# idthanm/mpg

Hardware: NVIDIA B200
Metric: model state-steps/s (fwd+bwd, n=25) (higher is better)
Workload: dtype f32

## Files before the change

### mpg_b200/csrc/api.cu

```cuda
#include <cstdio>
#include <cstdlib>
#include <cstring>
#include <new>
#include <vector>

#include "mlp_kernels.cuh"
#include "model_kernels.cuh"
#include "tc_rollout.cuh"
#include "replay.cuh"

using namespace mpg;

namespace {

struct NetStore {
  float* flat = nullptr;
  float* W1p = nullptr;
  float* W2p = nullptr;
  float* W2Tp = nullptr;
  float* adam_m = nullptr;
  float* adam_v = nullptr;
  int in_dim = 0, out_dim = 0;
  bool set = false;
};
// ... 541 lines not shown
  CUDA_OK(ctx, cudaMemcpyAsync(ns.adam_m, m, n * sizeof(float), cudaMemcpyDeviceToDevice, st));
  CUDA_OK(ctx, cudaMemcpyAsync(ns.adam_v, v, n * sizeof(float), cudaMemcpyDeviceToDevice, st));
  return MPG_OK;
}

int mpg_polyak_update(mpg_ctx* ctx, int src_net, int dst_net, float tau, void* stream) {
  int rc = check_net(ctx, src_net);
  if (!rc) rc = check_net(ctx, dst_net);
  if (rc) return rc;
  NetStore &a = ctx->nets[src_net], &d = ctx->nets[dst_net];
  if (a.in_dim != d.in_dim || a.out_dim != d.out_dim) return fail(ctx, MPG_ERR_ARG, "polyak: nets differ in shape%s");
  cudaStream_t st = (cudaStream_t)stream;
  const int n = layout(ctx, a).total;
  polyak_kernel<<<(n + 255) / 256, 256, 0, st>>>(d.flat, a.flat, n, tau);
  ctx->launches++;
  CUDA_OK(ctx, cudaGetLastError());
  return repack(ctx, dst_net, st);
}

int mpg_get_weights(mpg_ctx* ctx, int net, float* const w[6], void* stream) {
  int rc = check_net(ctx, net);
  if (rc) return rc;
  cudaStream_t st = (cudaStream_t)stream;
  NetStore& ns = ctx->nets[net];
  const GradLayout L = layout(ctx, ns);
  const int hw = ctx->cfg.hidden;
  const int off[6] = {L.oW1, L.ob1, L.oW2, L.ob2, L.oW3, L.ob3};
  const int cnt[6] = {ns.in_dim * hw, hw, hw * hw, hw, hw * ns.out_dim, ns.out_dim};
  for (int i = 0; i < 6; ++i)
    CUDA_OK(ctx, cudaMemcpyAsync(w[i], ns.flat + off[i], cnt[i] * sizeof(float), cudaMemcpyDefault, st));
  return MPG_OK;
}

int mpg_policy_grad(mpg_ctx* ctx, const mpg_rollout_params* p, const float* obs, const float* noise, float* grad_out,
                    float* returns_out, void* stream) {
  if (!ctx || !p || !obs || !grad_out) return fail(ctx, MPG_ERR_ARG, "null argument to mpg_policy_grad%s");
  if (p->real_env || ctx->cfg.env == MPG_ENV_PATH_TRACKING_REAL) return fail(ctx, MPG_ERR_UNSUPPORTED, "the real environment is forward only%s");
  cudaStream_t st = (cudaStream_t)stream;
  RolloutArgs a;
  int rc = fill_rollout_args(ctx, p, a);
  if (rc) return rc;
  a.obs = obs; a.noise = noise; a.returns_out = returns_out;
  a.noise_mode = noise ? 1 : (p->use_philox ? 2 : 0);
  const int MB = p->rows * p->M;
  if (ctx->backend == MPG_BACKEND_TC) {
    const int ntiles = (MB + tc::ACT_ROWS - 1) / tc::ACT_ROWS;
    const int grid = ntiles < ctx->sms ? ntiles : ctx->sms;
    tc::TcArgs ta = tc_args(ctx, a, p->policy_net, p->q_net);
    ta.store_steps = p->full_bptt ? p->horizon + 1 : 1;
    const size_t need = (size_t)ntiles * ta.store_steps * tc::SLOT_BYTES;
    if (!tc_ensure_store(ctx->tc, need)) return fail(ctx, MPG_ERR_CUDA, "cudaMalloc of the dW operand store failed%s");
    ta.store = ctx->tc.store;
    ta.rec_hi_only = rec_hi_only(ctx, (long long)MB * ta.store_steps);
    if (!tc_ensure_h2store(ctx->tc, (size_t)ntiles * (p->horizon + 1) * 2 * tc::ACT_SPLIT))
      return fail(ctx, MPG_ERR_CUDA, "cudaMalloc of the h2 image store failed%s");
    ta.h2store = ctx->tc.h2store;
    ta.z_ckpt = ctx->tc.z_ckpt;
    ta.prof = ctx->prof;
    const int tail = ntiles % ctx->sms, full = ntiles - tail;
    const bool split = ctx->tail_overlap && ctx->aux && full > 0 && tail > 0 && !ctx->prof
                       && (long long)(ctx->sms - tail) * 4 >= (long long)(full / ctx->sms) * ctx->sms / 2;
    CUDA_OK(ctx, cudaMemsetAsync(ctx->partial, 0, (size_t)(split ? 2 : 1) * ctx->sms * ctx->partial_stride * sizeof(float), st));
    if (ctx->timing) cudaEventRecord(ctx->ev0, st);
    if (!split) {
      CUDA_OK(ctx, tc_launch_rollout<true>(ctx->cfg.env, ctx->act, ta, grid, st));
      if (ctx->timing) { cudaEventRecord(ctx->ev1, st); ctx->timed = 1; }
      launch_dw(ctx, ta, 0, ntiles, 0, ctx->sms, st);
      launch_reduce(ctx, p->policy_net, ctx->sms, grad_out, nullptr, st);
      ctx->launches += 3;
    } else {
      ta.tile0 = 0; ta.tile1 = full;
      CUDA_OK(ctx, tc_launch_rollout<true>(ctx->cfg.env, ctx->act, ta, ctx->sms, st));
      CUDA_OK(ctx, cudaEventRecord(ctx->ev_wave, st));
      tc::TcArgs tb = ta;
      tb.tile0 = full; tb.tile1 = ntiles;
      tb.r.partial = ctx->partial + (size_t)ctx->sms * ctx->partial_stride;
      CUDA_OK(ctx, tc_launch_rollout<true>(ctx->cfg.env, ctx->act, tb, tail, st));
      if (ctx->timing) { cudaEventRecord(ctx->ev1, st); ctx->timed = 1; }
      CUDA_OK(ctx, cudaStreamWaitEvent(ctx->aux, ctx->ev_wave, 0));
      launch_dw(ctx, ta, 0, full, 0, ctx->sms - tail, ctx->aux);
      CUDA_OK(ctx, cudaEventRecord(ctx->ev_aux, ctx->aux));
      launch_dw(ctx, ta, full, tail, ctx->sms, ctx->sms, st);
      CUDA_OK(ctx, cudaStreamWaitEvent(st, ctx->ev_aux, 0));
      launch_reduce(ctx, p->policy_net, 2 * ctx->sms, grad_out, nullptr, st);
      ctx->launches += 5;
    }
    CUDA_OK(ctx, cudaGetLastError());
    return MPG_OK;
  }
  const int ntiles = (MB + TILE_R - 1) / TILE_R;
  const int grid = ntiles < ctx->sms ? ntiles : ctx->sms;
  CUDA_OK(ctx, cudaMemsetAsync(ctx->partial, 0, (size_t)grid * ctx->partial_stride * sizeof(float), st));
  rc = launch_rollout<true>(ctx, a, grid, st, ctx->cfg.env);
  if (rc) return rc;
  launch_reduce(ctx, p->policy_net, grid, grad_out, nullptr, st);
  ctx->launches++;
  CUDA_OK(ctx, cudaGetLastError());
  return MPG_OK;
}

int mpg_rollout_forward(mpg_ctx* ctx, const mpg_rollout_params* p, const float* obs, const float* start_actions,
                        const float* noise, float* returns_out, float* traj_obs, float* traj_rew, float* traj_act,
                        void* stream) {
  if (!ctx || !p || !obs) return fail(ctx, MPG_ERR_ARG, "null argument to mpg_rollout_forward%s");
  cudaStream_t st = (cudaStream_t)stream;
  RolloutArgs a;
  int rc = fill_rollout_args(ctx, p, a);
// ... 465 lines not shown
```

### mpg_b200/csrc/tc_common.cuh

```cuda
#pragma once
#include <cuda_bf16.h>
#include <cuda_fp16.h>

#include "common.cuh"

namespace mpg {
namespace tc {

constexpr int H = 256;

__device__ __forceinline__ uint32_t smem_u32(const void* p) { return (uint32_t)__cvta_generic_to_shared(p); }

__device__ __forceinline__ void mbar_init(uint64_t* bar, uint32_t count) {
  asm volatile("mbarrier.init.shared::cta.b64 [%0], %1;" ::"r"(smem_u32(bar)), "r"(count));
}
__device__ __forceinline__ void mbar_arrive(uint64_t* bar) {
  asm volatile("mbarrier.arrive.shared::cta.b64 _, [%0];" ::"r"(smem_u32(bar)) : "memory");
}
__device__ __forceinline__ void mbar_expect_tx(uint64_t* bar, uint32_t bytes) {
  asm volatile("mbarrier.arrive.expect_tx.shared::cta.b64 _, [%0], %1;" ::"r"(smem_u32(bar)), "r"(bytes) : "memory");
}
__device__ __forceinline__ bool mbar_try(uint64_t* bar, uint32_t parity) {
  uint32_t ok;
  asm volatile(
      "{\n\t.reg .pred p;\n\t"
      "mbarrier.try_wait.parity.shared::cta.b64 p, [%1], %2, %3;\n\t"
      "selp.u32 %0, 1, 0, p;\n\t}" : "=r"(ok) : "r"(smem_u32(bar)), "r"(parity), "r"(0x989680) : "memory");
  return ok != 0;
}
static __device__ unsigned long long* g_wait_dbg = nullptr;
#ifndef MPG_WAIT_LIMIT_CYCLES
#define MPG_WAIT_LIMIT_CYCLES 4000000000ll
#endif
static inline bool wait_dbg_attach(unsigned long long* dev_ptr) {
  return cudaMemcpyToSymbol(g_wait_dbg, &dev_ptr, sizeof(dev_ptr)) == cudaSuccess;
}
static __device__ __noinline__ void mbar_timeout(int site, uint32_t parity) {
  if (g_wait_dbg) {
    const int w = (int)(threadIdx.x >> 5);
    const int k = w >= 20 ? 5 + (w & 1) : w / 4;
    volatile unsigned long long* r = g_wait_dbg + 4 + 4 * k;
    r[0] = (unsigned long long)site;
    r[1] = (unsigned long long)blockIdx.x;
    r[2] = (unsigned long long)threadIdx.x;
    r[3] = (unsigned long long)parity + 1ull;
    g_wait_dbg[0] = 1ull;
    __threadfence_system();
  }
}
__device__ __forceinline__ void mbar_wait(uint64_t* bar, uint32_t parity, int site = 0) {
  if (mbar_try(bar, parity)) return;
  const long long t0 = clock64();
  while (!mbar_try(bar, parity)) {
    if (clock64() - t0 > MPG_WAIT_LIMIT_CYCLES) {
      mbar_timeout(site, parity);
      const long long t1 = clock64();
      while (clock64() - t1 < 400000000ll) {}
      __trap();
    }
  }
}
#define MBAR_WAIT(bar, parity) mbar_wait((bar), (parity), __LINE__)
__device__ __forceinline__ float ex2_ftz(float x) {
  float y;
  asm("ex2.approx.ftz.f32 %0, %1;" : "=f"(y) : "f"(x));
  return y;
}
__device__ __forceinline__ float exp_fast(float x) { return ex2_ftz(x * 1.4426950408889634f); }
__device__ __forceinline__ void fence_barrier_init() { asm volatile("fence.mbarrier_init.release.cluster;" ::: "memory"); }
__device__ __forceinline__ void fence_proxy_async() { asm volatile("fence.proxy.async.shared::cta;" ::: "memory"); }

__device__ __forceinline__ void bulk_g2s(void* smem_dst, const void* gmem_src, uint32_t bytes, uint64_t* bar) {
  asm volatile("cp.async.bulk.shared::cluster.global.mbarrier::complete_tx::bytes [%0], [%1], %2, [%3];" ::"r"(
                   smem_u32(smem_dst)), "l"(gmem_src), "r"(bytes), "r"(smem_u32(bar)) : "memory");
}
__device__ __forceinline__ void bulk_s2g(void* gmem_dst, const void* smem_src, uint32_t bytes) {
  asm volatile("cp.async.bulk.global.shared::cta.bulk_group [%0], [%1], %2;" ::"l"(gmem_dst), "r"(smem_u32(smem_src)),
               "r"(bytes) : "memory");
}
__device__ __forceinline__ void bulk_commit() { asm volatile("cp.async.bulk.commit_group;" ::: "memory"); }
__device__ __forceinline__ void bulk_wait_read_all() { asm volatile("cp.async.bulk.wait_group.read 0;" ::: "memory"); }
__device__ __forceinline__ void bulk_wait_read_pending(int pending) {
  switch (pending) {
    case 3: asm volatile("cp.async.bulk.wait_group.read 3;" ::: "memory"); break;
    case 2: asm volatile("cp.async.bulk.wait_group.read 2;" ::: "memory"); break;
    case 1: asm volatile("cp.async.bulk.wait_group.read 1;" ::: "memory"); break;
    default: asm volatile("cp.async.bulk.wait_group.read 0;" ::: "memory"); break;
  }
}
__device__ __forceinline__ void bulk_wait_all() { asm volatile("cp.async.bulk.wait_group 0;" ::: "memory"); }

__device__ __forceinline__ void tmem_alloc(uint32_t* smem_result, uint32_t ncols) {
  asm volatile("tcgen05.alloc.cta_group::1.sync.aligned.shared::cta.b32 [%0], %1;" ::"r"(smem_u32(smem_result)), "r"(ncols)
               : "memory");
  asm volatile("tcgen05.relinquish_alloc_permit.cta_group::1.sync.aligned;" ::: "memory");
}
__device__ __forceinline__ void tmem_dealloc(uint32_t taddr, uint32_t ncols) {
  asm volatile("tcgen05.dealloc.cta_group::1.sync.aligned.b32 %0, %1;" ::"r"(taddr), "r"(ncols) : "memory");
}
__device__ __forceinline__ void tc_fence_before() { asm volatile("tcgen05.fence::before_thread_sync;" ::: "memory"); }
__device__ __forceinline__ void tc_fence_after() { asm volatile("tcgen05.fence::after_thread_sync;" ::: "memory"); }

__device__ __forceinline__ void umma_bf16(uint32_t d_tmem, uint64_t a_desc, uint64_t b_desc, uint32_t idesc,
                                          uint32_t accumulate) {
  asm volatile(
      "{\n\t.reg .pred p;\n\t"
      "setp.ne.b32 p, %4, 0;\n\t"
      "tcgen05.mma.cta_group::1.kind::f16 [%0], %1, %2, %3, p;\n\t}" ::"r"(d_tmem), "l"(a_desc), "l"(b_desc), "r"(idesc),
      "r"(accumulate) : "memory");
}
__device__ __forceinline__ void umma_commit(uint64_t* bar) {
  asm volatile("tcgen05.commit.cta_group::1.mbarrier::arrive::one.shared::cluster.b64 [%0];" ::"r"(smem_u32(bar)) : "memory");
}

__device__ __forceinline__ void tmem_ld32(uint32_t taddr, float (&v)[32]) {
  uint32_t r[32];
  asm volatile(
      "tcgen05.ld.sync.aligned.32x32b.x32.b32 "
      "{%0, %1, %2, %3, %4, %5, %6, %7, %8, %9, %10, %11, %12, %13, %14, %15, "
      "%16, %17, %18, %19, %20, %21, %22, %23, %24, %25, %26, %27, %28, %29, %30, %31}, [%32];"
      : "=r"(r[0]), "=r"(r[1]), "=r"(r[2]), "=r"(r[3]), "=r"(r[4]), "=r"(r[5]), "=r"(r[6]), "=r"(r[7]), "=r"(r[8]),
        "=r"(r[9]), "=r"(r[10]), "=r"(r[11]), "=r"(r[12]), "=r"(r[13]), "=r"(r[14]), "=r"(r[15]), "=r"(r[16]),
        "=r"(r[17]), "=r"(r[18]), "=r"(r[19]), "=r"(r[20]), "=r"(r[21]), "=r"(r[22]), "=r"(r[23]), "=r"(r[24]),
        "=r"(r[25]), "=r"(r[26]), "=r"(r[27]), "=r"(r[28]), "=r"(r[29]), "=r"(r[30]), "=r"(r[31])
      : "r"(taddr));
  asm volatile("tcgen05.wait::ld.sync.aligned;" ::: "memory");
#pragma unroll
  for (int i = 0; i < 32; ++i) v[i] = __uint_as_float(r[i]);
}
__device__ __forceinline__ void tmem_ld16(uint32_t taddr, float (&v)[16]) {
  uint32_t r[16];
  asm volatile(
      "tcgen05.ld.sync.aligned.32x32b.x16.b32 "
// ... 91 lines not shown
```

### mpg_b200/csrc/tc_kernels.cuh

```cuda
#pragma once
#include "env_models.cuh"
#include "rollout_kernels.cuh"
#include "tc_gemm.cuh"

#ifndef MPG_EPI_INLINE
#define MPG_EPI_INLINE __forceinline__
#endif

namespace mpg {
namespace tc {

struct TcNet {
  const uint8_t* big_fwd;
  const uint8_t* big_dx;
  const uint8_t* l1;
  const uint8_t* l1b;
  const uint8_t* in;
  const float* W3;
  const float* b2;
  const float* b3;
  int in_dim, out_dim;
};

constexpr int BIAS_K = 15;
constexpr size_t SLOT_H1 = 0, SLOT_D2 = 131072, SLOT_P = 262144;
constexpr size_t SLOT_BYTES = 270336;

struct TcArgs {
  RolloutArgs r;
  TcNet pol, q;
  float* act_ckpt;
  float* z_ckpt;
  uint8_t* h2store;
  uint8_t* store;
  int store_steps;
  int rec_hi_only;
  int tile0, tile1;
  int q_regress;
  const float* q_target;
  float q_inv_rows;
  long long* prof;
};

struct MiscF {
  float W3p[H * 2];
  float b2p[H];
  float W3q[H * 2];
  float b2q[H];
  float part[4 * 2 * ACT_ROWS];
  float d3s[2 * ACT_ROWS];
  float wsum[8];
  float b3[4];
};
static_assert(sizeof(MiscF) <= SmemMap::MISC_BYTES, "MISC region too small");

constexpr int SM_D3IMG = SmemMap::TOTAL;
constexpr int SM_TOTAL = SM_D3IMG + 8192;

__device__ __forceinline__ void epi_bar() { asm volatile("bar.sync 1, %0;" ::"n"(EPI_THREADS) : "memory"); }
__device__ __forceinline__ float elu_fast(float x) { return x > 0.f ? x : exp_fast(x) - 1.f; }
template <int ACT>
__device__ __forceinline__ float act_fast(float x) {
  if constexpr (ACT == MPG_ACT_RELU) return x > 0.f ? x : 0.f;
  else if constexpr (ACT == MPG_ACT_TANH) return tanhf(x);
  else return elu_fast(x);
}
template <int ACT>
__device__ __forceinline__ float times_act_grad_out(float g, float h) {
  if constexpr (ACT == MPG_ACT_RELU) return h > 0.f ? g : 0.f;
  else if constexpr (ACT == MPG_ACT_TANH) return g * fmaf(-h, h, 1.f);
  else return fmaf(g, fminf(h, 0.f), g);
}
template <int ACT>
__device__ __forceinline__ float act_grad_log2e(float z) {
  if constexpr (ACT == MPG_ACT_RELU) {
    return z > 0.f ? 1.f : 0.f;
  } else if constexpr (ACT == MPG_ACT_TANH) {
    const float e = ex2_ftz(-2.f * fabsf(z)), d = 1.f + e;
    return __fdividef(4.f * e, d * d);
  } else {
    return ex2_ftz(fminf(z, 0.f));
  }
}

__device__ __forceinline__ void act_load8(const uint8_t* act_hi, const uint8_t* act_lo, int r, int cc, float* x) {
  const uint32_t off = act_chunk_off(r, cc);
  const uint4 h = *reinterpret_cast<const uint4*>(act_hi + off);
  const uint4 l = *reinterpret_cast<const uint4*>(act_lo + off);
  const uint32_t hw[4] = {h.x, h.y, h.z, h.w}, lw[4] = {l.x, l.y, l.z, l.w};
#pragma unroll
  for (int i = 0; i < 4; ++i) {
    x[2 * i] = __uint_as_float(hw[i] << 16) + __uint_as_float(lw[i] << 16);
    x[2 * i + 1] = __uint_as_float(hw[i] & 0xFFFF0000u) + __uint_as_float(lw[i] & 0xFFFF0000u);
  }
}

__device__ __forceinline__ void store_image(bool elected, uint8_t* gdst, const uint8_t* ssrc, uint32_t bytes) {
  fence_proxy_async();
  epi_bar();
  if (elected) {
    bulk_s2g(gdst, ssrc, bytes);
    bulk_commit();
  }
}
__device__ __forceinline__ void store_image_follow(bool elected, Bars* b, const Sync& s, uint8_t* gdst, const uint8_t* ssrc,
                                                   bool hi_only = false) {
  if (elected) {
    const uint32_t par = (s.k_cnt - 1) & 1;
#pragma unroll
    for (int kb = 0; kb < 4; ++kb) {
      mbar_wait(&b->kb_done[kb], par, 20000 + __LINE__);
// ... 178 lines not shown
}

__device__ __forceinline__ void bar_arrive(int id, int count) { asm volatile("bar.arrive %0, %1;" ::"r"(id), "r"(count) : "memory"); }
__device__ __forceinline__ void bar_sync(int id, int count) { asm volatile("bar.sync %0, %1;" ::"r"(id), "r"(count) : "memory"); }
constexpr int BAR_PART = 2;
constexpr int BAR_D3 = 3;
constexpr int BAR_ROW = 4;
constexpr int ROW_THREADS = ACT_ROWS;
constexpr int XCHG_THREADS = EPI_THREADS + ROW_THREADS;

template <int ENV, bool BWD, int ACT, int ROLE>
__device__ __forceinline__ void run_rollout(const TcArgs& A, uint8_t* smem, Bars* b) {
  using E = Env<ENV>;
  constexpr int S = E::S, NA = E::A;
  const RolloutArgs& a = A.r;
  const int tid = threadIdx.x, warp = tid >> 5, lane = tid & 31;
  const int row = (warp & 3) * 32 + lane, hc = (warp >> 2) & 3;
  const bool rowthread = (ROLE == ROLE_ROW);
  const bool elected = (ROLE == ROLE_EPI) && tid == 0;
  const int MB = a.rows * a.M;
  const int ntiles = (MB + ACT_ROWS - 1) / ACT_ROWS;
  MiscF* mf = reinterpret_cast<MiscF*>(smem + SmemMap::MISC);
  uint8_t* act_img = smem + SmemMap::ACT;
  uint8_t* p_img = smem + SmemMap::PIMG;
  uint8_t* d3_img = smem + SM_D3IMG;
  const uint32_t tmem = b->tmem_base;
  const uint32_t tm_z1c = tmem + TM_Z1C, tm_work = tmem + TM_WORK, tm_gp = tmem + TM_GP, tm_d1 = tmem + TM_D1, tm_d3 = tmem + TM_D3;
  const uint32_t lane_off = (uint32_t)((warp & 3) * 32) << 16;
  const float cscale = -1.f / ((float)a.M * (float)a.global_rows);
  const bool store_dw = BWD && A.store != nullptr;
  Sync sy;
  bool d1_started = false, d3_started = false;
  bool d1_pending = false, any_dw = false;
  bool store_pending = false;
  uint32_t acc_issued = 0;
  auto acc_wait = [&]() {
    if (ROLE == ROLE_ROW && d1_pending) {
      mbar_wait(&b->acc_done, sy.acc_cnt & 1, 20000 + __LINE__);
      ++sy.acc_cnt;
    }
    d1_pending = false;
  };
  float db3acc[2] = {0.f, 0.f};
  int prof_t = -1;
  auto stamp = [&](int id) {
#ifdef MPG_DEBUG_PROBES
    if (A.prof && blockIdx.x == 0 && prof_t >= 0
        && ((ROLE == ROLE_EPI && tid == 0) || ROLE == ROLE_MMA || (ROLE == ROLE_ROW && tid == EPI_THREADS)))
      A.prof[(ROLE == ROLE_MMA ? 32 : (ROLE == ROLE_ROW ? 64 : 0)) + id] = clock64();
#else
    (void)id; (void)prof_t;
#endif
  };

  unsigned long long list_bits = 0ull, q_bits = 0ull;
#pragma unroll
  for (int k = 0; k < MPG_MAX_LIST; ++k)
    if (k < a.n_list && a.list[k] < 64) {
      list_bits |= 1ull << a.list[k];
      if (a.list_w[k] != 0.f) q_bits |= 1ull << a.list[k];
    }
  auto list_index = [&](int tt) {
    int kidx = -1;
    if (tt >= 64 || ((list_bits >> tt) & 1ull)) {
#pragma unroll
      for (int k = 0; k < MPG_MAX_LIST; ++k) if (k < a.n_list && a.list[k] == tt) kidx = k;
    }
    return kidx;
  };

  const int tile_end = A.tile1 > 0 && A.tile1 < ntiles ? A.tile1 : ntiles;
  for (int tile = A.tile0 + blockIdx.x; tile < tile_end; tile += gridDim.x) {
    const int grow = tile * ACT_ROWS + row;
    const bool valid = rowthread && grow < MB;
    const int m_idx = valid ? grow / a.rows : 0, i_idx = valid ? grow % a.rows : 0;
    const unsigned long long noise_row = (unsigned long long)m_idx * (unsigned long long)a.global_rows
                                         + (unsigned long long)(a.row_offset + i_idx);
    uint8_t* h2tile = (BWD && A.h2store) ? A.h2store + (size_t)tile * (size_t)(a.horizon + 1) * (2 * ACT_SPLIT) : nullptr;
    float s[S];
#pragma unroll
    for (int j = 0; j < S; ++j) s[j] = 0.f;
    if (valid) {
      float o[MPG_MAX_OBS];
#pragma unroll
      for (int i = 0; i < MPG_MAX_OBS; ++i) o[i] = i < a.obs_dim ? a.obs[(size_t)i_idx * a.obs_dim + i] : 0.f;
      E::reset(o, s);
    }
    float rsum = 0.f, gpow = 1.f;

    auto write_pimg = [&](const float* st, const float* act_or_null, bool f16, uint8_t* gimg = nullptr) {
      float o[MPG_MAX_OBS];
#pragma unroll
      for (int i = 0; i < MPG_MAX_OBS; ++i) o[i] = 0.f;
      E::get_obs(st, o, a.nfd);
#pragma unroll
      for (int kh = 0; kh < 2; ++kh) {
        float x[8];
#pragma unroll
        for (int e = 0; e < 8; ++e) {
          const int i = kh * 8 + e;
          float v = i < a.obs_dim ? o[i] * a.obs_scale[i] : 0.f;
          if (act_or_null) {
#pragma unroll
            for (int j = 0; j < NA; ++j)
              if (i == a.obs_dim + j) v = act_or_null[j];
          }
          x[e] = i == BIAS_K ? 1.f : v;
        }
        uint4 h, l;
        if (f16) {
          split2h(x[0], x[1], h.x, l.x); split2h(x[2], x[3], h.y, l.y); split2h(x[4], x[5], h.z, l.z); split2h(x[6], x[7], h.w, l.w);
        } else {
          split2(x[0], x[1], h.x, l.x); split2(x[2], x[3], h.y, l.y); split2(x[4], x[5], h.z, l.z); split2(x[6], x[7], h.w, l.w);
        }
        const uint32_t off = p_chunk_off(row, kh);
        *reinterpret_cast<uint4*>(p_img + off) = h;
        *reinterpret_cast<uint4*>(p_img + off + P_LO) = l;
        if (gimg) {
          *reinterpret_cast<uint4*>(gimg + off) = h;
          *reinterpret_cast<uint4*>(gimg + off + P_LO) = l;
        }
      }
    };
    auto policy_forward = [&](float* zpre, uint8_t* h2slot, uint8_t* slot) {
      if (ROLE == ROLE_MMA) stamp(16);
#ifdef MPG_DEBUG_PROBES
      fwd_pair_issue<ROLE>(b, smem, sy, A.pol.l1, A.pol.big_fwd, tm_z1c, tm_work,
                           (ROLE == ROLE_MMA && A.prof && blockIdx.x == 0 && prof_t >= 0) ? A.prof + 96 : nullptr);
#else
      fwd_pair_issue<ROLE>(b, smem, sy, A.pol.l1, A.pol.big_fwd, tm_z1c, tm_work);
#endif
      if (ROLE == ROLE_MMA) stamp(17);
      if (ROLE == ROLE_EPI) {
        stamp(17);
        if (store_pending) { store_wait(elected); store_pending = false; }
        epi_hidden1_blocks<ACT>(b, tm_z1c + lane_off, act_img, row, hc);
        stamp(18);
        if (slot) { store_image_follow(elected, b, sy, slot + SLOT_H1, act_img, A.rec_hi_only != 0); store_pending = true; }
        epi_wait_d(b, sy);
        stamp(19);
        float p0, p1;
        if (BWD) epi_hidden2_gstore<ACT>(tm_work + lane_off, mf->b2p, mf->W3p, h2slot, row, hc, p0, p1);
        else epi_hidden2<ACT>(tm_work + lane_off, mf->b2p, mf->W3p, hc, p0, p1);
        stamp(20);
        mf->part[(hc * 2 + 0) * ACT_ROWS + row] = p0;
        mf->part[(hc * 2 + 1) * ACT_ROWS + row] = p1;
        bar_arrive(BAR_PART, XCHG_THREADS);
      }
      if (rowthread) {
        bar_sync(BAR_PART, XCHG_THREADS);
#pragma unroll
        for (int j = 0; j < NA; ++j)
          zpre[j] = mf->b3[j] + ((mf->part[(0 * 2 + j) * ACT_ROWS + row] + mf->part[(1 * 2 + j) * ACT_ROWS + row])
                                 + (mf->part[(2 * 2 + j) * ACT_ROWS + row] + mf->part[(3 * 2 + j) * ACT_ROWS + row]));
      }
    };
    auto q_forward = [&](bool with_img, uint8_t* qslot) -> float {
      float qv = 0.f;
      fwd_pair_issue<ROLE>(b, smem, sy, A.q.l1, A.q.big_fwd, tm_z1c, tm_work);
      if (ROLE == ROLE_EPI) {
        if (store_pending) { store_wait(elected); store_pending = false; }
        epi_hidden1_blocks<ACT>(b, tm_z1c + lane_off, act_img, row, hc);
        if (qslot) store_image(elected, qslot + SLOT_H1, act_img, A.rec_hi_only ? ACT_SPLIT : 2 * ACT_SPLIT);
        epi_wait_d(b, sy);
        float p0, p1;
        if (with_img) {
          if (qslot) store_wait(elected);
          epi_hidden2_img<ACT>(tm_work + lane_off, mf->b2q, mf->W3q, act_img, row, hc, p0, p1);
        } else {
          epi_hidden2<ACT>(tm_work + lane_off, mf->b2q, mf->W3q, hc, p0, p1);
        }
        mf->part[(hc * 2 + 0) * ACT_ROWS + row] = p0;
        bar_arrive(BAR_PART, XCHG_THREADS);
      }
      if (rowthread) {
        bar_sync(BAR_PART, XCHG_THREADS);
        qv = mf->b3[2] + ((mf->part[0 * ACT_ROWS + row] + mf->part[2 * ACT_ROWS + row])
                          + (mf->part[4 * ACT_ROWS + row] + mf->part[6 * ACT_ROWS + row]));
      }
      return qv;
    };

    acc_wait();
    for (int t = 0; t <= a.horizon; ++t) {
      float act[NA];
#pragma unroll
      for (int j = 0; j < NA; ++j) act[j] = 0.f;
      const bool given = (t == 0 && a.use_start_actions);
      const bool rec_f = store_dw && !A.q_regress && (a.full_bptt || t == 0);
      uint8_t* slot = rec_f ? A.store + ((size_t)tile * A.store_steps + (a.full_bptt ? t : 0)) * SLOT_BYTES : nullptr;
      if (tile == A.tile0 + (int)blockIdx.x && t == 2) {
        prof_t = t;
        if (ROLE != ROLE_MMA) stamp(16);
      } else if (prof_t >= 0) {
        if (ROLE != ROLE_MMA) stamp(22);
        prof_t = -1;
      }
      if (rowthread) {
        if (BWD && valid) {
          float* c = a.ckpt + ((size_t)t * MB + grow) * S;
#pragma unroll
          for (int j = 0; j < S; ++j) c[j] = s[j];
        }
        if (!given) write_pimg(s, nullptr, true);
      }
      if (!given) {
        float zpre[NA];
        policy_forward(zpre, BWD ? h2tile + (size_t)t * (2 * ACT_SPLIT) : nullptr, slot);
        stamp(21);
        if (rowthread) {
          float hg[NA];
#pragma unroll
          for (int j = 0; j < NA; ++j) head_fwd_grad(zpre[j], a.policy_out_tanh, a.action_range, act[j], hg[j]);
          if (BWD && valid)
#pragma unroll
            for (int j = 0; j < NA; ++j) {
              A.z_ckpt[((size_t)t * MB + grow) * (2 * NA) + j] = act[j];
              A.z_ckpt[((size_t)t * MB + grow) * (2 * NA) + NA + j] = hg[j];
            }
        }
      } else if (valid) {
#pragma unroll
        for (int j = 0; j < NA; ++j) act[j] = a.start_actions[(size_t)i_idx * NA + j];
      }
      if (valid && a.traj_act)
#pragma unroll
        for (int j = 0; j < NA; ++j) a.traj_act[((size_t)t * MB + grow) * NA + j] = act[j];
      const int kidx = list_index(t);
      if (kidx >= 0) {
        float qv = 0.f;
        if (BWD && valid)
#pragma unroll
          for (int j = 0; j < NA; ++j) A.act_ckpt[((size_t)kidx * MB + grow) * NA + j] = act[j];
        if (a.has_q) {
          if (rowthread) write_pimg(s, act, true);
          qv = q_forward(false, nullptr);
        }
        if (valid && a.returns_out)
#pragma unroll
          for (int k = 0; k < MPG_MAX_LIST; ++k)
            if (k < a.n_list && a.list[k] == t) a.returns_out[(size_t)k * MB + grow] = rsum + gpow * qv;
      }
      if (t < a.horizon && valid) {
        float eps = 0.f;
        if (E::HAS_NOISE) {
          if (a.noise_mode == 1) eps = a.noise[(size_t)t * MB + grow];
          else if (a.noise_mode == 2) eps = philox_normal(a.seed, noise_row, (uint32_t)t);
        }
        const float rew = E::step(s, act, eps, a.noise_mode != 0);
        const float prew = (rew + a.rew_shift) * a.rew_scale;
        rsum += gpow * prew;
        gpow *= a.gamma;
        if (a.traj_rew) a.traj_rew[(size_t)t * MB + grow] = prew;
        if (a.traj_obs) {
          float o[MPG_MAX_OBS];
          E::get_obs(s, o, a.nfd);
#pragma unroll
          for (int i = 0; i < MPG_MAX_OBS; ++i)
            if (i < a.obs_dim) a.traj_obs[((size_t)t * MB + grow) * a.obs_dim + i] = o[i];
        }
      }
    }
    if (BWD) {
      float lam[S], snext[S], spre[S], zpre_n[2 * NA];
#pragma unroll
      for (int j = 0; j < S; ++j) { lam[j] = 0.f; snext[j] = s[j]; spre[j] = s[j]; }
#pragma unroll
      for (int j = 0; j < 2 * NA; ++j)
        zpre_n[j] = (valid && !A.q_regress) ? A.z_ckpt[((size_t)a.horizon * MB + grow) * (2 * NA) + j] : 0.f;
      float w_later = 0.f;
      for (int t = a.horizon; t >= 0; --t) {
        if (t < a.horizon && list_index(t + 1) >= 0) {
#pragma unroll
          for (int k = 0; k < MPG_MAX_LIST; ++k) if (k < a.n_list && a.list[k] == t + 1) w_later += a.list_w[k];
        }
        float gp = 1.f;
        for (int i = 0; i < t; ++i) gp *= a.gamma;
        const bool want_dw = a.full_bptt || t == 0;
        const bool rec = store_dw && want_dw;
        prof_t = (tile == A.tile0 + (int)blockIdx.x && t == a.horizon - 2) ? t : -1;
        stamp(0);
        uint8_t* slot = rec ? A.store + ((size_t)tile * A.store_steps + (a.full_bptt ? t : 0)) * SLOT_BYTES : nullptr;
        float g_a[NA], g_s[S], act[NA], hgrad[NA];
#pragma unroll
        for (int j = 0; j < NA; ++j) { g_a[j] = 0.f; act[j] = zpre_n[j]; hgrad[j] = zpre_n[NA + j]; }
#pragma unroll
        for (int j = 0; j < S; ++j) g_s[j] = 0.f;
        if (valid) {
#pragma unroll
          for (int j = 0; j < S; ++j) s[j] = spre[j];
          if (t > 0) {
            const float* c = a.ckpt + ((size_t)(t - 1) * MB + grow) * S;
#pragma unroll
            for (int j = 0; j < S; ++j) spre[j] = c[j];
            if (!A.q_regress)
#pragma unroll
              for (int j = 0; j < 2 * NA; ++j) zpre_n[j] = A.z_ckpt[((size_t)(t - 1) * MB + grow) * (2 * NA) + j];
          }
        }
        if (ROLE == ROLE_ROW) stamp(4);
        const int kidx = list_index(t);
        if (want_dw) any_dw = true;
        float w_k = 0.f;
        if (kidx >= 0) {
#pragma unroll
          for (int k = 0; k < MPG_MAX_LIST; ++k) if (k < a.n_list && a.list[k] == t) w_k += a.list_w[k];
        }
        auto q_part_at = [&](int tt) {
          bool q = false;
          if (tt < 64) {
            q = (q_bits >> tt) & 1ull;
          } else {
#pragma unroll
            for (int k = 0; k < MPG_MAX_LIST; ++k) if (k < a.n_list && a.list[k] == tt && a.list_w[k] != 0.f) q = true;
          }
          return q && a.has_q;
        };
        const bool early = t < a.horizon && !q_part_at(t);
        const bool early_next = t > 0 && !q_part_at(t - 1) && !A.q_regress;
        auto load_h2 = [&](int tt) {
          const uint8_t* src = h2tile + (size_t)tt * (2 * ACT_SPLIT);
#pragma unroll
          for (int h = 0; h < 2; ++h) {
            mbar_wait(&b->img_empty[h], sy.i_cnt & 1, 20000 + __LINE__);
            mbar_expect_tx(&b->img_full[h], ACT_SPLIT);
#pragma unroll
            for (int sp = 0; sp < 2; ++sp)
#pragma unroll
              for (int k = 0; k < 2; ++k) {
                const size_t off = (size_t)sp * ACT_SPLIT + (size_t)(2 * h + k) * ACT_BLOCK;
                bulk_g2s(act_img + off, src + off, ACT_BLOCK, &b->img_full[h]);
              }
          }
        };
        if (kidx >= 0 && a.has_q && (q_part_at(t) || A.q_regress)) {
          const bool reg = A.q_regress != 0;
          uint8_t* qslot = (reg && store_dw) ? A.store + (size_t)tile * SLOT_BYTES : nullptr;
          if (rowthread) {
            float ak[NA];
#pragma unroll
            for (int j = 0; j < NA; ++j) ak[j] = valid ? A.act_ckpt[((size_t)kidx * MB + grow) * NA + j] : 0.f;
            acc_wait();
            write_pimg(s, ak, true);
          }
          const float qv = q_forward(true, qslot);
          if (rowthread) {
            float ak[NA];
#pragma unroll
            for (int j = 0; j < NA; ++j) ak[j] = valid ? A.act_ckpt[((size_t)kidx * MB + grow) * NA + j] : 0.f;
            write_pimg(s, ak, false, qslot ? qslot + SLOT_P : nullptr);
            fence_proxy_async();
            mbar_arrive(&b->p_full);
          }
          if (rowthread) {
            const float up = !valid ? 0.f : (reg ? (qv - A.q_target[i_idx]) * A.q_inv_rows : cscale * w_k * gp);
            mf->d3s[row] = up;
            if (reg) {
              write_d3(d3_img, row, up, 0.f);
              db3acc[0] += up;
            }
            bar_arrive(BAR_D3, XCHG_THREADS);
          }
          if (reg) d3_issue<ROLE>(b, smem, sy, SM_D3IMG, d3_started, tm_d3);
          if (ROLE == ROLE_EPI) {
            if (reg) epi_wait_d(b, sy);
            bar_sync(BAR_D3, XCHG_THREADS);
          }
          gemm_issue<ROLE>(0, b, smem, sy, A.q.big_dx, tm_work);
          if (ROLE == ROLE_EPI) {
            epi_delta2_blocks<ACT>(b, mf->W3q, mf->d3s[row], 0.f, act_img, row, hc, reg ? &sy : nullptr);
            if (qslot) store_image(elected, qslot + SLOT_D2, act_img, A.rec_hi_only ? ACT_SPLIT : 2 * ACT_SPLIT);
            epi_wait_d(b, sy);
          }
          bwd_tail_issue<ROLE>(b, smem, sy, A.q.l1b, A.q.in, !reg, reg, d1_started, tm_z1c, tm_gp, tm_d1, true);
          if (ROLE == ROLE_EPI) {
            if (qslot) store_wait(elected);
            epi_delta1_blocks<ACT>(b, tm_work + lane_off, tm_z1c + lane_off, act_img, row, hc);
            if (!reg) epi_wait_d(b, sy);
          }
          if (reg) { d1_pending = true; ++acc_issued; }
          if (rowthread && !reg) {
            mbar_wait(&b->gp_full, sy.gp_cnt & 1, 20000 + __LINE__);
            ++sy.gp_cnt;
            tc_fence_after();
            float gin[16];
            read_gp(tm_gp + lane_off, gin);
            if (valid) {
              float go[MPG_MAX_OBS];
#pragma unroll
              for (int i = 0; i < MPG_MAX_OBS; ++i) go[i] = i < a.obs_dim ? gin[i] * a.obs_scale[i] : 0.f;
              E::obs_grad_to_state(s, go, a.nfd, g_s);
#pragma unroll
              for (int j = 0; j < NA; ++j)
#pragma unroll
                for (int i = 0; i < 16; ++i)
                  if (i == a.obs_dim + j) g_a[j] += gin[i];
            }
          }
        }
        if (A.q_regress) continue;
        if (rowthread) {
          tc_fence_before();
          stamp(5);
          if (t < a.horizon && valid) {
            env_step_bwd<ENV, true>(s, act, lam, cscale * w_later * gp * a.rew_scale, g_s, g_a, snext);
          }
          stamp(14);
          float d3[2] = {0.f, 0.f};
#pragma unroll
          for (int j = 0; j < NA; ++j) {
            d3[j] = valid ? g_a[j] * hgrad[j] : 0.f;
            mf->d3s[j * ACT_ROWS + row] = d3[j];
          }
          if (NA == 1) mf->d3s[ACT_ROWS + row] = 0.f;
          if (want_dw) {
            write_d3(d3_img, row, d3[0], d3[1]);
            db3acc[0] += d3[0]; db3acc[1] += d3[1];
          }
          bar_arrive(BAR_D3, XCHG_THREADS);
          stamp(2);
        }
        if (!early) {
          if (ROLE == ROLE_MMA) { umma_commit(&b->img_empty[0]); umma_commit(&b->img_empty[1]); }
          if (elected) {
            bulk_wait_read_all();
            mbar_arrive(&b->img_empty[0]);
            mbar_arrive(&b->img_empty[1]);
          }
          if (ROLE == ROLE_PRODUCER) load_h2(t);
        }
        store_pending = false;
        stamp(1);
        if (ROLE == ROLE_EPI) {
          mbar_wait(&b->img_full[0], sy.i_cnt & 1, 20000 + __LINE__);
          stamp(3);
        }
        ++sy.i_cnt;
        if (ROLE == ROLE_MMA) stamp(5);
        if (want_dw) d3_issue<ROLE>(b, smem, sy, SM_D3IMG, d3_started, tm_d3, true, A.rec_hi_only != 0);
        if (ROLE == ROLE_MMA) stamp(6);
        if (rowthread) {
          acc_wait();
          stamp(12);
          write_pimg(s, nullptr, false, rec ? slot + SLOT_P : nullptr);
          fence_proxy_async();
          mbar_arrive(&b->p_full);
          stamp(13);
        }
        if (ROLE == ROLE_EPI) {
          bar_sync(BAR_D3, XCHG_THREADS);
        }
        if (ROLE == ROLE_MMA) stamp(3);
        gemm_issue<ROLE>(0, b, smem, sy, A.pol.big_dx, tm_work);
        if (ROLE == ROLE_MMA) stamp(4);
        if (ROLE == ROLE_EPI) {
          stamp(6);
          epi_delta2_from_h2<ACT>(b, mf->W3p, mf->d3s[row], mf->d3s[ACT_ROWS + row], act_img, row, hc, (sy.i_cnt - 1) & 1,
                             want_dw ? &sy : nullptr);
          stamp(7);
          if (rec) store_image_follow(elected, b, sy, slot + SLOT_D2, act_img, A.rec_hi_only != 0);
          epi_wait_d(b, sy);
          stamp(8);
        }
        bwd_tail_issue<ROLE>(b, smem, sy, A.pol.l1b, A.pol.in, t > 0, want_dw, d1_started, tm_z1c, tm_gp, tm_d1, true, early_next);
        if (ROLE == ROLE_PRODUCER && early_next) load_h2(t - 1);
        if (ROLE == ROLE_EPI) {
          epi_delta1_blocks<ACT>(b, tm_work + lane_off, tm_z1c + lane_off, act_img, row, hc, rec, elected, early_next);
          stamp(9);
          if (t > 0) epi_wait_d(b, sy);
          stamp(10);
        }
        if (want_dw) { d1_pending = true; ++acc_issued; }
        if (t > 0 && rowthread) {
          mbar_wait(&b->gp_full, sy.gp_cnt & 1, 20000 + __LINE__);
          ++sy.gp_cnt;
          tc_fence_after();
          stamp(10);
          float gin[16];
          read_gp(tm_gp + lane_off, gin);
          if (valid) {
#pragma unroll
            for (int j = 0; j < S; ++j) { lam[j] = g_s[j]; snext[j] = s[j]; }
            float go[MPG_MAX_OBS];
#pragma unroll
            for (int i = 0; i < MPG_MAX_OBS; ++i) go[i] = i < a.obs_dim ? gin[i] * a.obs_scale[i] : 0.f;
            E::obs_grad_to_state(s, go, a.nfd, lam);
          }
        }
        stamp(11);
      }
    }
  }
  if (rowthread && BWD) {
    float s0 = db3acc[0], s1 = db3acc[1];
#pragma unroll
    for (int o = 16; o > 0; o >>= 1) { s0 += __shfl_xor_sync(0xffffffffu, s0, o); s1 += __shfl_xor_sync(0xffffffffu, s1, o); }
    if (lane == 0) { mf->wsum[(warp & 3) * 2] = s0; mf->wsum[(warp & 3) * 2 + 1] = s1; }
    bar_sync(BAR_ROW, ROW_THREADS);
    if (tid == EPI_THREADS) {
      const GradLayout L(A.pol.in_dim, A.pol.out_dim, H);
      float* partial = a.partial + (size_t)blockIdx.x * a.partial_stride;
      partial[L.ob3 + 0] = (mf->wsum[0] + mf->wsum[2]) + (mf->wsum[4] + mf->wsum[6]);
      if (NA > 1) partial[L.ob3 + 1] = (mf->wsum[1] + mf->wsum[3]) + (mf->wsum[5] + mf->wsum[7]);
    }
  }
  if (ROLE == ROLE_EPI && acc_issued > 0) mbar_wait(&b->acc_done, (acc_issued - 1) & 1, 20000 + __LINE__);
  if (ROLE == ROLE_EPI) {
    tc_fence_before();
    if (elected) bulk_wait_all();
    if (BWD) {
      const GradLayout L(A.pol.in_dim, A.pol.out_dim, H);
      float* partial = a.partial + (size_t)blockIdx.x * a.partial_stride;
      if (any_dw && hc == 0) {
        tc_fence_after();
        const int ncol3 = A.q_regress ? 1 : NA;
#pragma unroll
        for (int half = 0; half < 2; ++half) {
          const int f = half * 128 + row;
          float v[16], v2[16];
          tmem_ld16(tm_d1 + half * 32 + lane_off, v);
          tmem_ld16(tm_d1 + half * 32 + 16 + lane_off, v2);
#pragma unroll
          for (int i = 0; i < 16; ++i)
            if (i < A.pol.in_dim) partial[L.oW1 + (size_t)i * H + f] = v[i] + v2[i];
          partial[L.ob1 + f] = v[BIAS_K] + v2[BIAS_K];
          tmem_ld16(tm_d3 + half * 16 + lane_off, v);
#pragma unroll
          for (int j = 0; j < 2; ++j)
            if (j < ncol3) partial[L.oW3 + (size_t)f * A.pol.out_dim + j] = v[j] + v[2 + j];
        }
      }
    }
  }
}

constexpr int ROLLOUT_THREADS = EPI_THREADS + ROW_THREADS + 128;
constexpr int ROW_WARP0 = EPI_WARPS, PRODUCER_WARP = EPI_WARPS + 4, MMA_WARP = EPI_WARPS + 5;
constexpr int LAUNCH_REGS = 80, EPI_REGS = 80, ROW_REGS = 96, AUX_REGS = 64;
static_assert(EPI_THREADS * EPI_REGS + ROW_THREADS * ROW_REGS + 128 * AUX_REGS <= ROLLOUT_THREADS * LAUNCH_REGS,
              "setmaxnreg only redistributes the register pool of the CTA");

template <int ENV, bool BWD, int ACT>
__global__ void __launch_bounds__(ROLLOUT_THREADS, 1) tc_rollout_kernel(const __grid_constant__ TcArgs A) {
  extern __shared__ uint8_t smem_raw[];
// ... 36 lines not shown
```

Measured before the change: 635.5 million.

## Cache Q-net hidden images in forward and prefetch them in backward pass

During the forward rollout, the Q-network's second-layer hidden activations at list steps are now written to an extended global h2 store. The backward pass then reloads them by bulk copy and recomputes only the delta from h2, instead of rerunning the Q forward GEMMs at those steps. The image pipeline is restructured so every backward step, including Q steps, prefetches the next image early, and the weights for upcoming forward passes are warmed in L2. The change also adds debug-gated timing probes, and in exchange uses more global memory and adds proxy fences.

```diff
diff --git a/mpg_b200/csrc/api.cu b/mpg_b200/csrc/api.cu
--- a/mpg_b200/csrc/api.cu
+++ b/mpg_b200/csrc/api.cu
@@ -617,7 +617,7 @@
     if (!tc_ensure_store(ctx->tc, need)) return fail(ctx, MPG_ERR_CUDA, "cudaMalloc of the dW operand store failed%s");
     ta.store = ctx->tc.store;
     ta.rec_hi_only = rec_hi_only(ctx, (long long)MB * ta.store_steps);
-    if (!tc_ensure_h2store(ctx->tc, (size_t)ntiles * (p->horizon + 1) * 2 * tc::ACT_SPLIT))
+    if (!tc_ensure_h2store(ctx->tc, (size_t)ntiles * (p->horizon + 1 + p->n_list) * 2 * tc::ACT_SPLIT))
       return fail(ctx, MPG_ERR_CUDA, "cudaMalloc of the h2 image store failed%s");
     ta.h2store = ctx->tc.h2store;
     ta.z_ckpt = ctx->tc.z_ckpt;
diff --git a/mpg_b200/csrc/tc_common.cuh b/mpg_b200/csrc/tc_common.cuh
--- a/mpg_b200/csrc/tc_common.cuh
+++ b/mpg_b200/csrc/tc_common.cuh
@@ -69,6 +69,7 @@
 __device__ __forceinline__ float exp_fast(float x) { return ex2_ftz(x * 1.4426950408889634f); }
 __device__ __forceinline__ void fence_barrier_init() { asm volatile("fence.mbarrier_init.release.cluster;" ::: "memory"); }
 __device__ __forceinline__ void fence_proxy_async() { asm volatile("fence.proxy.async.shared::cta;" ::: "memory"); }
+__device__ __forceinline__ void fence_proxy_async_global() { asm volatile("fence.proxy.async.global;" ::: "memory"); }
 
 __device__ __forceinline__ void bulk_g2s(void* smem_dst, const void* gmem_src, uint32_t bytes, uint64_t* bar) {
   asm volatile("cp.async.bulk.shared::cluster.global.mbarrier::complete_tx::bytes [%0], [%1], %2, [%3];" ::"r"(
@@ -79,6 +80,9 @@
                "r"(bytes) : "memory");
 }
 __device__ __forceinline__ void bulk_commit() { asm volatile("cp.async.bulk.commit_group;" ::: "memory"); }
+__device__ __forceinline__ void prefetch_l2(const void* gsrc, uint32_t bytes) {
+  asm volatile("cp.async.bulk.prefetch.L2.global [%0], %1;" ::"l"(gsrc), "r"(bytes) : "memory");
+}
 __device__ __forceinline__ void bulk_wait_read_all() { asm volatile("cp.async.bulk.wait_group.read 0;" ::: "memory"); }
 __device__ __forceinline__ void bulk_wait_read_pending(int pending) {
   switch (pending) {
diff --git a/mpg_b200/csrc/tc_kernels.cuh b/mpg_b200/csrc/tc_kernels.cuh
--- a/mpg_b200/csrc/tc_kernels.cuh
+++ b/mpg_b200/csrc/tc_kernels.cuh
@@ -42,6 +42,12 @@
   long long* prof;
 };
 
+constexpr int ACCT_TILE0 = 0, ACCT_FWD0 = 1, ACCT_BWD0 = 2, ACCT_TILE1 = 3, ACCT_NS0 = 4, ACCT_NS1 = 5;
+constexpr int ACCT_FSTEP = 8, ACCT_FQ = 72, ACCT_BSTEP = 136, ACCT_BQ = 200, ACCT_BMID = 264;
+constexpr int PROF_ACCT = 128, PROF_ACCT_STRIDE = 336;
+constexpr int PROF_TILES = PROF_ACCT + 2 * 3 * PROF_ACCT_STRIDE, PROF_TILES_MAX = 16;
+constexpr int PROF_LONGLONGS = PROF_TILES + 2 * PROF_TILES_MAX * 4;
+
 struct MiscF {
   float W3p[H * 2];
   float b2p[H];
@@ -57,6 +63,11 @@
 constexpr int SM_D3IMG = SmemMap::TOTAL;
 constexpr int SM_TOTAL = SM_D3IMG + 8192;
 
+__device__ __forceinline__ unsigned long long globaltimer_ns() {
+  unsigned long long t;
+  asm volatile("mov.u64 %0, %%globaltimer;" : "=l"(t));
+  return t;
+}
 __device__ __forceinline__ void epi_bar() { asm volatile("bar.sync 1, %0;" ::"n"(EPI_THREADS) : "memory"); }
 __device__ __forceinline__ float elu_fast(float x) { return x > 0.f ? x : exp_fast(x) - 1.f; }
 template <int ACT>
@@ -341,6 +352,22 @@
     (void)id; (void)prof_t;
 #endif
   };
+#ifdef MPG_DEBUG_PROBES
+  const int acct_slot = !A.prof ? -1 : (blockIdx.x == 0 ? 0 : (blockIdx.x == gridDim.x / 2 ? 1 : -1));
+  const bool acct_thread = (ROLE == ROLE_EPI && tid == 0) || ROLE == ROLE_MMA || (ROLE == ROLE_ROW && tid == EPI_THREADS);
+  long long* acct = (acct_slot >= 0 && acct_thread)
+                        ? A.prof + PROF_ACCT + (acct_slot * 3 + (ROLE == ROLE_EPI ? 0 : (ROLE == ROLE_MMA ? 1 : 2))) * PROF_ACCT_STRIDE
+                        : nullptr;
+  bool acct_on = false;
+#endif
+  auto astamp = [&](int id) {
+#ifdef MPG_DEBUG_PROBES
+    if (acct && acct_on) acct[id] = clock64();
+#else
+    (void)id;
+#endif
+  };
+  auto astamp_step = [&](int base, int tt) { if (tt < 64) astamp(base + tt); };
 
   unsigned long long list_bits = 0ull, q_bits = 0ull;
 #pragma unroll
@@ -357,15 +384,45 @@
     }
     return kidx;
   };
+  auto q_part_at = [&](int tt) {
+    bool q = false;
+    if (tt < 64) {
+      q = (q_bits >> tt) & 1ull;
+    } else {
+#pragma unroll
+      for (int k = 0; k < MPG_MAX_LIST; ++k) if (k < a.n_list && a.list[k] == tt && a.list_w[k] != 0.f) q = true;
+    }
+    return q && a.has_q;
+  };
+  auto warm_fwd_l2 = [&](const TcNet& n) {
+    if (ROLE == ROLE_PRODUCER && BWD && !A.q_regress) {
+      for (int i = 0; i < BIG_STAGES; ++i) prefetch_l2(n.big_fwd + (size_t)i * STAGE_BYTES, STAGE_BYTES);
+      prefetch_l2(n.l1, STAGE_BYTES);
+    }
+  };
 
   const int tile_end = A.tile1 > 0 && A.tile1 < ntiles ? A.tile1 : ntiles;
   for (int tile = A.tile0 + blockIdx.x; tile < tile_end; tile += gridDim.x) {
+#ifdef MPG_DEBUG_PROBES
+    const int tile_i = (tile - A.tile0 - (int)blockIdx.x) / (int)gridDim.x;
+    acct_on = tile_i == (tile_end - A.tile0 - (int)blockIdx.x > (int)gridDim.x ? 1 : 0);
+    if (acct && acct_on) acct[ACCT_NS0] = (long long)globaltimer_ns();
+    if (acct_slot >= 0 && elected && tile_i < PROF_TILES_MAX) {
+      long long* tl = A.prof + PROF_TILES + (acct_slot * PROF_TILES_MAX + tile_i) * 4;
+      tl[0] = clock64();
+      tl[1] = (long long)globaltimer_ns();
+    }
+#endif
+    astamp(ACCT_TILE0);
     const int grow = tile * ACT_ROWS + row;
     const bool valid = rowthread && grow < MB;
     const int m_idx = valid ? grow / a.rows : 0, i_idx = valid ? grow % a.rows : 0;
     const unsigned long long noise_row = (unsigned long long)m_idx * (unsigned long long)a.global_rows
                                          + (unsigned long long)(a.row_offset + i_idx);
     uint8_t* h2tile = (BWD && A.h2store) ? A.h2store + (size_t)tile * (size_t)(a.horizon + 1) * (2 * ACT_SPLIT) : nullptr;
+    auto h2q_img = [&](int kk) {
+      return A.h2store + ((size_t)ntiles * (size_t)(a.horizon + 1) + (size_t)tile * a.n_list + kk) * (2 * ACT_SPLIT);
+    };
     float s[S];
 #pragma unroll
     for (int j = 0; j < S; ++j) s[j] = 0.f;
@@ -444,7 +501,7 @@
                                  + (mf->part[(2 * 2 + j) * ACT_ROWS + row] + mf->part[(3 * 2 + j) * ACT_ROWS + row]));
       }
     };
-    auto q_forward = [&](bool with_img, uint8_t* qslot) -> float {
+    auto q_forward = [&](bool with_img, uint8_t* qslot, uint8_t* h2slot = nullptr) -> float {
       float qv = 0.f;
       fwd_pair_issue<ROLE>(b, smem, sy, A.q.l1, A.q.big_fwd, tm_z1c, tm_work);
       if (ROLE == ROLE_EPI) {
@@ -456,6 +513,8 @@
         if (with_img) {
           if (qslot) store_wait(elected);
           epi_hidden2_img<ACT>(tm_work + lane_off, mf->b2q, mf->W3q, act_img, row, hc, p0, p1);
+        } else if (BWD && h2slot) {
+          epi_hidden2_gstore<ACT>(tm_work + lane_off, mf->b2q, mf->W3q, h2slot, row, hc, p0, p1);
         } else {
           epi_hidden2<ACT>(tm_work + lane_off, mf->b2q, mf->W3q, hc, p0, p1);
         }
@@ -471,7 +530,10 @@
     };
 
     acc_wait();
+    astamp(ACCT_FWD0);
     for (int t = 0; t <= a.horizon; ++t) {
+      astamp_step(ACCT_FSTEP, t);
+      if (t < a.horizon && q_part_at(t + 1)) warm_fwd_l2(A.q);
       float act[NA];
 #pragma unroll
       for (int j = 0; j < NA; ++j) act[j] = 0.f;
@@ -522,8 +584,9 @@
 #pragma unroll
           for (int j = 0; j < NA; ++j) A.act_ckpt[((size_t)kidx * MB + grow) * NA + j] = act[j];
         if (a.has_q) {
+          astamp_step(ACCT_FQ, t);
           if (rowthread) write_pimg(s, act, true);
-          qv = q_forward(false, nullptr);
+          qv = q_forward(false, nullptr, (BWD && h2tile && !A.q_regress && q_part_at(t)) ? h2q_img(kidx) : nullptr);
         }
         if (valid && a.returns_out)
 #pragma unroll
@@ -550,6 +613,7 @@
         }
       }
     }
+    astamp(ACCT_BWD0);
     if (BWD) {
       float lam[S], snext[S], spre[S], zpre_n[2 * NA];
 #pragma unroll
@@ -558,6 +622,35 @@
       for (int j = 0; j < 2 * NA; ++j)
         zpre_n[j] = (valid && !A.q_regress) ? A.z_ckpt[((size_t)a.horizon * MB + grow) * (2 * NA) + j] : 0.f;
       float w_later = 0.f;
+      auto bwd_img = [&](int tt) { return q_part_at(tt) ? h2q_img(list_index(tt)) : h2tile + (size_t)tt * (2 * ACT_SPLIT); };
+      auto load_img = [&](const uint8_t* src) {
+#pragma unroll
+        for (int h = 0; h < 2; ++h) {
+          mbar_wait(&b->img_empty[h], sy.i_cnt & 1, 20000 + __LINE__);
+          mbar_expect_tx(&b->img_full[h], ACT_SPLIT);
+#pragma unroll
+          for (int sp = 0; sp < 2; ++sp)
+#pragma unroll
+            for (int k = 0; k < 2; ++k) {
+              const size_t off = (size_t)sp * ACT_SPLIT + (size_t)(2 * h + k) * ACT_BLOCK;
+              bulk_g2s(act_img + off, src + off, ACT_BLOCK, &b->img_full[h]);
+            }
+        }
+      };
+      if (!A.q_regress) {
+        if (ROLE == ROLE_MMA) { umma_commit(&b->img_empty[0]); umma_commit(&b->img_empty[1]); }
+        if (ROLE == ROLE_EPI) {
+          fence_proxy_async_global();
+          epi_bar();
+        }
+        if (elected) {
+          bulk_wait_read_all();
+          mbar_arrive(&b->img_empty[0]);
+          mbar_arrive(&b->img_empty[1]);
+        }
+        store_pending = false;
+        if (ROLE == ROLE_PRODUCER) load_img(bwd_img(a.horizon));
+      }
       for (int t = a.horizon; t >= 0; --t) {
         if (t < a.horizon && list_index(t + 1) >= 0) {
 #pragma unroll
@@ -569,6 +662,11 @@
         const bool rec = store_dw && want_dw;
         prof_t = (tile == A.tile0 + (int)blockIdx.x && t == a.horizon - 2) ? t : -1;
         stamp(0);
+        astamp_step(ACCT_BSTEP, t);
+        if (t == 1 && tile + (int)gridDim.x < tile_end) {
+          warm_fwd_l2(A.pol);
+          if (q_part_at(0)) warm_fwd_l2(A.q);
+        }
         uint8_t* slot = rec ? A.store + ((size_t)tile * A.store_steps + (a.full_bptt ? t : 0)) * SLOT_BYTES : nullptr;
         float g_a[NA], g_s[S], act[NA], hgrad[NA];
 #pragma unroll
@@ -595,44 +693,23 @@
 #pragma unroll
           for (int k = 0; k < MPG_MAX_LIST; ++k) if (k < a.n_list && a.list[k] == t) w_k += a.list_w[k];
         }
-        auto q_part_at = [&](int tt) {
-          bool q = false;
-          if (tt < 64) {
-            q = (q_bits >> tt) & 1ull;
-          } else {
-#pragma unroll
-            for (int k = 0; k < MPG_MAX_LIST; ++k) if (k < a.n_list && a.list[k] == tt && a.list_w[k] != 0.f) q = true;
-          }
-          return q && a.has_q;
-        };
-        const bool early = t < a.horizon && !q_part_at(t);
-        const bool early_next = t > 0 && !q_part_at(t - 1) && !A.q_regress;
-        auto load_h2 = [&](int tt) {
-          const uint8_t* src = h2tile + (size_t)tt * (2 * ACT_SPLIT);
-#pragma unroll
-          for (int h = 0; h < 2; ++h) {
-            mbar_wait(&b->img_empty[h], sy.i_cnt & 1, 20000 + __LINE__);
-            mbar_expect_tx(&b->img_full[h], ACT_SPLIT);
-#pragma unroll
-            for (int sp = 0; sp < 2; ++sp)
-#pragma unroll
-              for (int k = 0; k < 2; ++k) {
-                const size_t off = (size_t)sp * ACT_SPLIT + (size_t)(2 * h + k) * ACT_BLOCK;
-                bulk_g2s(act_img + off, src + off, ACT_BLOCK, &b->img_full[h]);
-              }
-          }
-        };
+        const bool early_next = t > 0 && !A.q_regress;
         if (kidx >= 0 && a.has_q && (q_part_at(t) || A.q_regress)) {
           const bool reg = A.q_regress != 0;
           uint8_t* qslot = (reg && store_dw) ? A.store + (size_t)tile * SLOT_BYTES : nullptr;
-          if (rowthread) {
-            float ak[NA];
-#pragma unroll
-            for (int j = 0; j < NA; ++j) ak[j] = valid ? A.act_ckpt[((size_t)kidx * MB + grow) * NA + j] : 0.f;
+          float qv = 0.f;
+          if (reg) {
+            if (rowthread) {
+              float ak[NA];
+#pragma unroll
+              for (int j = 0; j < NA; ++j) ak[j] = valid ? A.act_ckpt[((size_t)kidx * MB + grow) * NA + j] : 0.f;
+              acc_wait();
+              write_pimg(s, ak, true);
+            }
+            qv = q_forward(true, qslot);
+          } else if (rowthread) {
             acc_wait();
-            write_pimg(s, ak, true);
-          }
-          const float qv = q_forward(true, qslot);
+          }
           if (rowthread) {
             float ak[NA];
 #pragma unroll
@@ -653,18 +730,22 @@
           if (reg) d3_issue<ROLE>(b, smem, sy, SM_D3IMG, d3_started, tm_d3);
           if (ROLE == ROLE_EPI) {
             if (reg) epi_wait_d(b, sy);
+            else mbar_wait(&b->img_full[0], sy.i_cnt & 1, 20000 + __LINE__);
             bar_sync(BAR_D3, XCHG_THREADS);
           }
+          if (!reg) ++sy.i_cnt;
           gemm_issue<ROLE>(0, b, smem, sy, A.q.big_dx, tm_work);
           if (ROLE == ROLE_EPI) {
-            epi_delta2_blocks<ACT>(b, mf->W3q, mf->d3s[row], 0.f, act_img, row, hc, reg ? &sy : nullptr);
+            if (reg) epi_delta2_blocks<ACT>(b, mf->W3q, mf->d3s[row], 0.f, act_img, row, hc, &sy);
+            else epi_delta2_from_h2<ACT>(b, mf->W3q, mf->d3s[row], 0.f, act_img, row, hc, (sy.i_cnt - 1) & 1);
             if (qslot) store_image(elected, qslot + SLOT_D2, act_img, A.rec_hi_only ? ACT_SPLIT : 2 * ACT_SPLIT);
             epi_wait_d(b, sy);
           }
-          bwd_tail_issue<ROLE>(b, smem, sy, A.q.l1b, A.q.in, !reg, reg, d1_started, tm_z1c, tm_gp, tm_d1, true);
+          bwd_tail_issue<ROLE>(b, smem, sy, A.q.l1b, A.q.in, !reg, reg, d1_started, tm_z1c, tm_gp, tm_d1, true, !reg);
+          if (ROLE == ROLE_PRODUCER && !reg) load_img(h2tile + (size_t)t * (2 * ACT_SPLIT));
           if (ROLE == ROLE_EPI) {
             if (qslot) store_wait(elected);
-            epi_delta1_blocks<ACT>(b, tm_work + lane_off, tm_z1c + lane_off, act_img, row, hc);
+            epi_delta1_blocks<ACT>(b, tm_work + lane_off, tm_z1c + lane_off, act_img, row, hc, false, elected, !reg);
             if (!reg) epi_wait_d(b, sy);
           }
           if (reg) { d1_pending = true; ++acc_issued; }
@@ -686,6 +767,7 @@
                   if (i == a.obs_dim + j) g_a[j] += gin[i];
             }
           }
+          astamp_step(ACCT_BQ, t);
         }
         if (A.q_regress) continue;
         if (rowthread) {
@@ -708,21 +790,13 @@
           }
           bar_arrive(BAR_D3, XCHG_THREADS);
           stamp(2);
-        }
-        if (!early) {
-          if (ROLE == ROLE_MMA) { umma_commit(&b->img_empty[0]); umma_commit(&b->img_empty[1]); }
-          if (elected) {
-            bulk_wait_read_all();
-            mbar_arrive(&b->img_empty[0]);
-            mbar_arrive(&b->img_empty[1]);
-          }
-          if (ROLE == ROLE_PRODUCER) load_h2(t);
-        }
-        store_pending = false;
+          astamp_step(ACCT_BMID, t);
+        }
         stamp(1);
         if (ROLE == ROLE_EPI) {
           mbar_wait(&b->img_full[0], sy.i_cnt & 1, 20000 + __LINE__);
           stamp(3);
+          astamp_step(ACCT_BMID, t);
         }
         ++sy.i_cnt;
         if (ROLE == ROLE_MMA) stamp(5);
@@ -739,7 +813,7 @@
         if (ROLE == ROLE_EPI) {
           bar_sync(BAR_D3, XCHG_THREADS);
         }
-        if (ROLE == ROLE_MMA) stamp(3);
+        if (ROLE == ROLE_MMA) { stamp(3); astamp_step(ACCT_BMID, t); }
         gemm_issue<ROLE>(0, b, smem, sy, A.pol.big_dx, tm_work);
         if (ROLE == ROLE_MMA) stamp(4);
         if (ROLE == ROLE_EPI) {
@@ -752,7 +826,7 @@
           stamp(8);
         }
         bwd_tail_issue<ROLE>(b, smem, sy, A.pol.l1b, A.pol.in, t > 0, want_dw, d1_started, tm_z1c, tm_gp, tm_d1, true, early_next);
-        if (ROLE == ROLE_PRODUCER && early_next) load_h2(t - 1);
+        if (ROLE == ROLE_PRODUCER && early_next) load_img(bwd_img(t - 1));
         if (ROLE == ROLE_EPI) {
           epi_delta1_blocks<ACT>(b, tm_work + lane_off, tm_z1c + lane_off, act_img, row, hc, rec, elected, early_next);
           stamp(9);
@@ -779,6 +853,15 @@
         stamp(11);
       }
     }
+    astamp(ACCT_TILE1);
+#ifdef MPG_DEBUG_PROBES
+    if (acct && acct_on) acct[ACCT_NS1] = (long long)globaltimer_ns();
+    if (acct_slot >= 0 && elected && tile_i < PROF_TILES_MAX) {
+      long long* tl = A.prof + PROF_TILES + (acct_slot * PROF_TILES_MAX + tile_i) * 4;
+      tl[2] = clock64();
+      tl[3] = (long long)globaltimer_ns();
+    }
+#endif
   }
   if (rowthread && BWD) {
     float s0 = db3acc[0], s1 = db3acc[1];
```

Result: no change. 640.8 million (median of 6 runs) (+0.8%).
